# thisparticle/scl_slam

Hardware: AMD Instinct MI355X
Metric: loop-closure candidates/sec: (scan, keyframe) pairs taken through full-database ARG-MIN detection per second (every pair aligned exactly and bounded by the f16 matrix-core screening; only the survivors get the f64 distance), batches of 16 scans, 10k-keyframe DB per GPU (higher is better)
Workload: dtype f64 results; f16-operand / f32-accumulate MFMA screening + f64 exact pass on the survivors

## Files before the change

profiles/summarize_pmc.py:

```python
import collections
import csv
import glob
import json
import sys


def summarize(root, needle):
    agg = collections.defaultdict(list)
    for f in glob.glob(f"{root}/**/*_counter_collection.csv", recursive=True):
        for row in csv.DictReader(open(f)):
            if needle in row["Kernel_Name"]:
                agg[row["Counter_Name"]].append(float(row["Counter_Value"]))
    summary = {k: {"launches": len(v), "mean_per_launch": sum(v) / len(v)} for k, v in sorted(agg.items())}
    res = {"kernel_filter": needle, "counters": summary}
    if "FETCH_SIZE" in summary and "WRITE_SIZE" in summary:
        fetch = summary["FETCH_SIZE"]["mean_per_launch"] * 1024.0 * 2.0
        write = summary["WRITE_SIZE"]["mean_per_launch"] * 1024.0
        res["hbm_bytes_per_launch"] = fetch + write
        res["hbm_read_bytes_corrected_x2"] = fetch
        res["hbm_write_bytes"] = write
    return res


def main():
    root, out = sys.argv[1], sys.argv[2]
    needles = (sys.argv[3] if len(sys.argv) > 3 else "sc_distance").split(",")
    if len(needles) == 1:
        res = summarize(root, needles[0])
    else:
        parts = [summarize(root, n) for n in needles]
        res = {"kernel_filter": needles, "kernels": parts}
        if all("hbm_bytes_per_launch" in p for p in parts):
            res["hbm_bytes_per_launch"] = sum(p["hbm_bytes_per_launch"] for p in parts)
            res["hbm_read_bytes_corrected_x2"] = sum(p["hbm_read_bytes_corrected_x2"] for p in parts)
            res["hbm_write_bytes"] = sum(p["hbm_write_bytes"] for p in parts)
    json.dump(res, open(out, "w"), indent=1)
    print(json.dumps(res, indent=1))


if __name__ == "__main__":
    main()
# ... 1 lines not shown
```

scl_slam_amd/csrc/engine.hip:

```cpp
#include "scl_engine.h"

#include <hip/hip_runtime.h>

#include <cfloat>
#include <climits>
#include <chrono>
#include <cmath>
#include <cstdio>
#include <cstdlib>
#include <cstring>
#include <mutex>
#include <new>
#include <string>
#include <atomic>
#include <chrono>
#include <thread>
#include <vector>

#include "db_file.hpp"
#include "engine_internal.hpp"
#include "device_sort.hpp"
#include "plugin_host.hpp"

#ifdef SCL_DIAGNOSTICS
// ... 451 lines not shown
    if (!c) return SCL_ERR_INVALID_ARG;
    c->num_ring = 20; c->num_sector = 60; c->num_candidates = 3;
    c->dist_thres = 0.14; c->lidar_height = 1.65; c->max_radius = 80.0;
    c->num_exclude_recent = 100; c->tree_making_period = 10;
    c->search_ratio = 0.1;
    c->knn_exclude_eps = 0.0f;
    c->device = 0;
    c->initial_capacity = 4096;
    return SCL_OK;
}

static void log_env_overrides_once()
{
    static std::atomic<bool> done{false};
    if (done.exchange(true)) return;
    static const char *const names[] = {"SCL_SCREEN", "SCL_SCREEN_FORM", "SCL_SCREEN_V2_MIN", "SCL_RCCL_LIB",
                                        "SCL_SCREEN_VARIANT", "SCL_SCREEN_PROBE", "SCL_SCREEN_TAIL", "SCL_ALIGN_WGS",
                                        "SCL_ALIGN2_WGS", "SCL_ALIGN_FILTER", "SCL_SC_KERNEL", "SCL_SC_WAVES", "SCL_STAMP", "SCL_ABLATE",
                                        "SCL_ICP_REDUCE", "SCL_MATRIX_PLAIN", "SCL_MATRIX_KERNEL", "SCL_MATRIX_KR", "SCL_WIDE_EXACT", "SCL_STREAM_EXACT", "SCL_SMALL_EXACT_OFF",
                                        "SCL_SELF_ALIGN_OFF", "SCL_CAND_EXACT_OFF"};
    constexpr int kProduct = 4;
    int i = 0;
    for (const char *n : names) {
        const char *v = getenv(n);
#ifdef SCL_DIAGNOSTICS
        if (v) fprintf(stderr, "scl_engine (diagnostics build): environment override in effect: %s=%s\n", n, v);
#else
        if (v && i < kProduct) fprintf(stderr, "scl_engine: environment override in effect: %s=%s\n", n, v);
        else if (v) fprintf(stderr, "scl_engine: %s=%s is an experiment's switch: ignored by this build (make EXTRA=-DSCL_DIAGNOSTICS builds them in)\n", n, v);
#endif
        ++i;
    }
    (void)kProduct;
}

int scl_create(const scl_config *cfg, scl_engine **out)
// ... 779 lines not shown
int scl_sc_search_inter(scl_engine *e, const int *curs, int count, int robot_pre, int k, int *cand_ids, int *cand_shifts, double *cand_dists,
                        int *n_found)
{
    if (!e || count < 0 || k < 1 || k > SCL_SC_SEARCH_MAX || (count > 0 && (!curs || !cand_ids))) return SCL_ERR_INVALID_ARG;
    if (robot_pre < SCL_SC_ANY_OTHER_ROBOT || robot_pre > 127) return SCL_ERR_INVALID_ARG;
    if (count == 0) return SCL_OK;
    if (e->front) return front_sc_search_inter(e, curs, count, robot_pre, k, cand_ids, cand_shifts, cand_dists, n_found);
    return sc_search_robot(e, curs, count, true, robot_pre, k, cand_ids, cand_shifts, cand_dists, n_found);
}

namespace {

int submit_full_many_locked(scl_engine *e, const int *queries, const int *los, const int *his, int nq, int *tickets);

struct ScreenGroup { const int *qslot, *lo, *n; int nq, set0; int part_half = 0; bool masks = false; bool keys_later = false; };
int launch_screen_group(scl_engine *e, const ScreenGroup &cur, int phases = kScreenAlign | kScreenProducts,
                        const ScreenGroup *next = nullptr, hipStream_t stream = nullptr)
{
    if (!stream) stream = e->stream;
    auto fill = [&](ScreenBatch &sb, const ScreenGroup &g) {
        sb.nq = g.nq;
        for (int j = 0; j < g.nq; ++j) { sb.slot[j] = g.qslot[j]; sb.base[j] = g.lo[j]; sb.n[j] = g.n[j]; sb.buf[j] = g.set0 + j; }
        sb.pair_stride = e->set_stride;
        sb.approx = e->d_approx; sb.starts = e->d_starts; sb.align_fallbacks = e->d_align_fallbacks; sb.ring_d2 = e->d_ring_d2;
        sb.survivors = nullptr; sb.n_surv = nullptr; sb.t_min = e->d_tmin;
        sb.smask = (g.masks || sc_screen_is_wide(db_view(e), e->SR)) ? e->d_smask : nullptr;
        sb.part = e->d_part + (g.part_half ? e->part_cap / 2 : 0);
        sb.no_ring_metric = g.keys_later;
        sb.k = e->cfg.num_candidates; sb.exclude_eps = e->cfg.knn_exclude_eps; sb.topk_idx = e->d_topk_idx; sb.topk_d2 = e->d_topk_d2;
    };
    ScreenBatch sb{}, nx{};
    fill(sb, cur);
    const bool has_next = next && next->nq > 0;
    if (has_next) fill(nx, *next);
    if (phases & kScreenAlign) for (int j = 0; j < cur.nq; ++j) e->align_pairs += (uint64_t)cur.n[j];
    if (has_next) for (int j = 0; j < next->nq; ++j) e->align_pairs += (uint64_t)next->n[j];
    if ((phases & kScreenAlign) && (phases & kScreenProducts) && has_next) {
        SCL_HIP(e, launch_sc_screen_batch(db_view(e), sb, e->SR, sc_align_filter_enabled(), e->num_cu, stream, kScreenAlign, nullptr));
        phases = kScreenProducts;
    }
    ProfScope ps(e, P_SC, stream);
    SCL_HIP(e, launch_sc_screen_batch(db_view(e), sb, e->SR, sc_align_filter_enabled(), e->num_cu, stream, phases, has_next ? &nx : nullptr));
    if (ps.active()) { for (int j = 0; j < cur.nq; ++j) e->prof.sc_distance_pairs += (uint64_t)cur.n[j]; }
    return SCL_OK;
}

unsigned survivor_arg_region(scl_engine *e) { return e->surv_arg_tick++ & 7u; }
int launch_survivor_pass(scl_engine *e, const int *qslot, const int *lo, const int *n, int nq, int set0, double *const *out3, hipStream_t stream = nullptr,
                         int phases = kSurvivorArgs | kSurvivorKernel, int region_in = -1, bool ring_from_keys = false)
{
    if (!stream) stream = e->stream;
    SurvivorPass sp{};
    sp.nq = nq; sp.ring_from_keys = ring_from_keys ? 1 : 0;
    for (int j = 0; j < nq; ++j) { sp.slot[j] = qslot[j]; sp.base[j] = lo[j]; sp.n[j] = n[j]; sp.buf[j] = set0 + j; sp.out3[j] = out3[j]; }
    sp.pair_stride = e->set_stride;
    sp.approx = e->d_approx; sp.survivors = e->d_surv; sp.t_min = e->d_tmin; sp.out_dist = e->d_dist; sp.out_shift = e->d_shift;
    sp.blk_part = e->d_surv_part; sp.done_counter = e->d_surv_done; sp.surv_stats = e->d_surv_stats;
    sp.ring_d2 = e->d_ring_d2; sp.k = e->cfg.num_candidates; sp.exclude_eps = e->cfg.knn_exclude_eps; sp.topk_idx = e->d_topk_idx; sp.topk_d2 = e->d_topk_d2;
// ... 366 lines not shown

int stream_screened_locked(scl_engine *e, std::unique_lock<std::mutex> &db, const int *queries, const int *lo, const int *hi, int n_queries, int spl,
                           int *nn_idx, int *shift, double *dist)
{
    const int n0 = e->n;
    constexpr int NS = scl_engine::kScreenSets;
    constexpr int CH = NS / 2;
    static_assert(CH <= kMaxSurvivorQueries, "one exact pass takes the survivors of a whole chunk");
    const bool wide = sc_screen_is_wide(db_view(e), e->SR);
#ifndef SCL_WIDE_CHUNK
#define SCL_WIDE_CHUNK 64
#endif
    const int chmax = wide && CH > SCL_WIDE_CHUNK ? SCL_WIDE_CHUNK : CH;
    const int chn = spl >= 1 && spl <= chmax ? (chmax / spl) * spl : chmax;
    struct List { int qslot[CH], qlo[CH], qn[CH], pos[CH], m = 0; };
    struct Chunk { int first = 0, count = 0; bool busy = false, aligned = false, small = false; std::vector<int> lo, empty; };
    Chunk ch[2];
    bool sub0_valid[2] = {false, false};
    const bool small_exact = sc_small_exact_supported(db_view(e), e->SR) && (!wide || e->d_smask) && !scl_lab_is("SCL_STREAM_EXACT", "s");
    const bool keys_later = !wide && !small_exact;
    int nmax = 1;
    for (int i = 0; i < n_queries; ++i) {
        const int l = lo[i] < 0 ? 0 : lo[i], h = hi[i] > n0 ? n0 : hi[i];
        if (h - l > nmax) nmax = h - l;
    }
    int rc = ensure_sets(e, (size_t)nmax);
    if (rc) return rc;
    SCL_HIP(e, hipEventRecord(e->ev_align_gate, e->stream));
    SCL_HIP(e, hipStreamWaitEvent(e->stream_surv, e->ev_align_gate, 0));
    auto build = [&](int first, int count, List &L, Chunk *k) -> int {
        L.m = 0;
        for (int i = 0; i < count; ++i) {
            const int q = queries[first + i];
            int slot;
            if (q >= 0) { if (q >= n0) return fail(e, SCL_ERR_OUT_OF_RANGE, "query slot out of range"); slot = q; }
// ... 27 lines not shown
        if (e->prof_on == 3 && cur.m > 0) {
            if ((e->prof_tick++ & 1) == 0) {
                auto get = [&]() { hipEvent_t ev = nullptr; if (!e->event_pool.empty()) { ev = e->event_pool.back(); e->event_pool.pop_back(); } else if (hipEventCreate(&ev) != hipSuccess) ev = nullptr; return ev; };
                span_start = get(); span_stop = get();
                if (span_start && span_stop) (void)hipEventRecord(span_start, e->stream); else { span_start = span_stop = nullptr; }
            }
            e->prof_on = 0;
        }
        auto span_end = [&]() {
            if (!span_start) return;
            (void)hipEventRecord(span_stop, e->stream);
            e->pending.push_back({span_start, span_stop, P_SC, span_groups});
            for (int j = 0; j < cur.m; ++j) e->prof.sc_distance_pairs += (uint64_t)cur.qn[j];
            span_start = nullptr;
        };
        bool next_aligned = false;
        for (int g = 0; g < cur.m; g += spl) {
            const int w = cur.m - g < spl ? cur.m - g : spl;
            ScreenGroup grp{cur.qslot + g, cur.qlo + g, cur.qn + g, w, set0 + g};
            grp.keys_later = keys_later;
            ScreenGroup nx{nullptr, nullptr, nullptr, 0, 0};
            if (g + w < cur.m) {
                const int wn = cur.m - g - w < spl ? cur.m - g - w : spl;
                nx = ScreenGroup{cur.qslot + g + w, cur.qlo + g + w, cur.qn + g + w, wn, set0 + g + w};
                nx.keys_later = keys_later;
            } else if (ncount > 0 && nxt.m > 0) {
                const int wn = nxt.m < spl ? nxt.m : spl;
                nx = ScreenGroup{nxt.qslot, nxt.qlo, nxt.qn, wn, nset0};
                nx.keys_later = keys_later;
                if (ch[c ^ 1].busy) SCL_HIP(e, hipStreamWaitEvent(e->stream, (wide && sub0_valid[c ^ 1] && wn <= kWideExactBatch) ? e->ev_sub0[c ^ 1] : e->ev_chunk[c ^ 1], 0));
                next_aligned = true;
            }
            const int phases = (g == 0 && !k.aligned) ? (kScreenAlign | kScreenProducts) : kScreenProducts;
            if ((rc = launch_screen_group(e, grp, phases, nx.nq > 0 ? &nx : nullptr))) return rc;
            ++span_groups;
        }
        span_end();
        hipStream_t xs = ncount > 0 ? e->stream_surv : e->stream;
        if (ncount > 0) {
            SCL_HIP(e, hipEventRecord(e->ev_k1[c], e->stream));
            SCL_HIP(e, hipStreamWaitEvent(e->stream_surv, e->ev_k1[c], 0));
        } else if (cur.m > 0) {
            if (hipEventQuery(e->ev_k1[c]) != hipSuccess) SCL_HIP(e, hipStreamWaitEvent(e->stream, e->ev_k1[c], 0));
        }
        sub0_valid[c] = wide && !k.small && cur.m > 0;
        if (cur.m > 0 && (rc = k.small ? launch_small_exact_chunk(e, cur.qslot, cur.qlo, cur.qn, cur.m, set0, out3, xs, kSurvivorKernel, region)
                             : wide ? launch_survivor_pass_wide(e, cur.qslot, cur.qlo, cur.qn, cur.m, set0, out3, xs, e->ev_sub0[c])
                                    : launch_survivor_pass(e, cur.qslot, cur.qlo, cur.qn, cur.m, set0, out3, xs, kSurvivorKernel, region, keys_later))) return rc;
        SCL_HIP(e, hipEventRecord(e->ev_chunk[c], xs));
        k.busy = true;
        k.aligned = false;
        ch[c ^ 1].aligned = next_aligned;
        e->last_pass_empty = cur.m == 0;
        return SCL_OK;
    };
    auto collect = [&](int c, bool last) -> int {
        Chunk &k = ch[c];
        auto wait_chunk = [&]() -> hipError_t {
            hipError_t q;
            const auto t0 = std::chrono::steady_clock::now();
            int spins = 0;
            while ((q = hipEventQuery(e->ev_chunk[c])) == hipErrorNotReady) {
                for (int p = 0; p < 32; ++p) cpu_relax();
                if ((++spins & 255) == 0 && std::chrono::steady_clock::now() - t0 > std::chrono::milliseconds(20)) return hipEventSynchronize(e->ev_chunk[c]);
            }
            return q;
// ... 2253 lines not shown
```

scl_slam_amd/csrc/kernels.hpp:

```cpp
#pragma once

#include <hip/hip_runtime.h>
#include <stdint.h>

#include <stdlib.h>

namespace scl {

#ifdef SCL_DIAGNOSTICS
inline int scl_lab_int(const char *name, int dflt) { const char *e = getenv(name); return e ? atoi(e) : dflt; }
inline bool scl_lab_is(const char *name, const char *value) { const char *e = getenv(name); if (!e) return false; while (*value) if (*e++ != *value++) return false; return true; }
#else
constexpr int scl_lab_int(const char *, int dflt) { return dflt; }
constexpr bool scl_lab_is(const char *, const char *) { return false; }
#endif

constexpr double kBigDist = 10000000.0;
constexpr int kTminEpsOffset = 256;
constexpr int hdesc_sector(int RG) { return ((RG * 8 + 63) / 64) * 8; }
constexpr int hkey_halfs(int S) { return ((S + 31) / 32) * 32; }
constexpr int hkey_store_halfs(int S) { return hkey_halfs(S) + 8; }
constexpr int hkey_row_halfs(int S) { return 2 * hkey_halfs(S) + 8; }
constexpr int halign_P(int S) { return S % 8 == 0 ? 8 : (S % 4 == 0 ? 4 : 0); }
constexpr int halign_CP(int S) { return ((S + 8 + 31) / 32) * 32; }
// ... 116 lines not shown
    unsigned long long *align_fallbacks;
    unsigned long long *surv_stats;
    unsigned int *smask;
    int k; float exclude_eps; int *topk_idx; float *topk_d2;
    float *part;
    bool no_ring_metric;
};
bool sc_screen_supported(const struct DbView &db, int SR);
bool sc_screen_is_wide(const struct DbView &db, int SR);
float sc_screen_eps();
int sc_screen_max_batch(const struct DbView &db, int SR);
size_t sc_screen_scratch_floats(const struct DbView &db, int SR);
constexpr int kScreenAlign = 1, kScreenProducts = 2;
hipError_t launch_sc_screen_batch(const struct DbView &db, const ScreenBatch &sb, int SR, int align_filter, int num_cu, hipStream_t stream,
                                  int phases = kScreenAlign | kScreenProducts, const ScreenBatch *next = nullptr);
hipError_t launch_sc_select_batch(const ScreenBatch &sb, hipStream_t stream);
constexpr int kSurvivorBlocks = 2;
constexpr int kSurvivorArgBytes = 384;
constexpr int kMaxSurvivorQueries = 128;
struct SurvivorPass {
    int nq;
    int slot[kMaxSurvivorQueries], base[kMaxSurvivorQueries], n[kMaxSurvivorQueries], buf[kMaxSurvivorQueries];
    double *out3[kMaxSurvivorQueries];
    size_t pair_stride;
    const float *approx; int *survivors; unsigned int *t_min; double *out_dist; int *out_shift;
    const float *ring_d2; int k; float exclude_eps; int *topk_idx; float *topk_d2;
    unsigned long long *blk_part; unsigned int *done_counter;
    unsigned long long *surv_stats;
    void *d_args; void *h_args;
    int ring_from_keys;
// ... 62 lines not shown
```

scl_slam_amd/csrc/sc_screen.hip:

```cpp
#include <atomic>
#include <type_traits>

#include "align_exact.hpp"
#include "device_common.hpp"
#include "kernels.hpp"

namespace scl {

namespace {

typedef _Float16 h4 __attribute__((ext_vector_type(4)));
typedef _Float16 h8 __attribute__((ext_vector_type(8)));
typedef float f4v __attribute__((ext_vector_type(4)));
typedef float f2 __attribute__((ext_vector_type(2)));
typedef unsigned int u32x4 __attribute__((ext_vector_type(4)));
typedef u32x4 __attribute__((aligned(8))) u32x4_a8;

struct ScreenArgs {
    const double *vkey;
    const uint2 *hdesc; const unsigned int *kmask;
    const double *q_vkey; const float *q_rkey;
    const uint2 *q_hdesc; const unsigned int *q_kmask;
    const _Float16 *hkey; const _Float16 *q_hkey; int hkw;
    const float4 *rkey4; int rk_cap;
// ... 947 lines not shown
    using C = S2Cfg<RG, S, W>;
    return (size_t)(C::NQ / (4 * C::SPK)) * s2_quad(S, C::STEPS * C::SPK, C::SPK);
}
template <int RG, int S, int W> constexpr bool s2_group_used(int p, int g4) { return 4 * g4 < kS2PassRows && W - 1 - S2Cfg<RG, S, W>::PS * p - 4 * g4 >= 0; }
template <int RG, int S, int W> constexpr int s2_pass_f4(int p) { int n = 0; for (int g = 0; g < 4; ++g) n += s2_group_used<RG, S, W>(p, g) ? 1 : 0; return n; }
template <int RG, int S, int W> constexpr int s2_pass_off(int p) { int o = 0; for (int q = 0; q < p; ++q) o += s2_pass_f4<RG, S, W>(q); return o; }
template <int RG, int S, int W> constexpr int s2_part_f4() { return s2_pass_off<RG, S, W>(S2Cfg<RG, S, W>::NPASS); }
template <int RG, int S, int W> constexpr int s2_part_floats() { return S2Cfg<RG, S, W>::NP * s2_part_f4<RG, S, W>() * 4; }

struct Screen2Args {
    ScreenBatchArgs prod;
    float *part;
    int u_lo, u_n;
    int nwg;
};

template <int RG, int S, int W>
__global__ __launch_bounds__((S2Cfg<RG, S, W>::WV * kWave), 1) void sc_screen2_kernel(Screen2Args fa)
{
    using C = S2Cfg<RG, S, W>;
    constexpr int WVP = C::WV;
    constexpr int NP = C::NP, NPASS = C::NPASS, STEPS = C::STEPS, NQ = C::NQ, SPK = C::SPK, PS = C::PS;
    constexpr bool AOFF = PS != kS2PassRows;
    constexpr int NB = AOFF ? 1 : NPASS;
    constexpr int LAG = AOFF ? PS / 4 : 0;
    constexpr int RGH = hdesc_rgh(RG);
    constexpr int SB = RGH * 8;
    constexpr int HS = hdesc_stride(RG, S);
    constexpr int SECT = STEPS * SPK;
    constexpr int NIT = S / SECT;
    constexpr int ROWS = S + SECT - 1;
    constexpr int QUAD = s2_quad(S, SECT, SPK);
    constexpr int SPR = 4 * SPK, SCB = 64 / SPK;
    static_assert(SB >= SCB * NP && SB == 64 * ((NP * SCB + 63) / 64) && S % SECT == 0 && SECT == 4 && kS2PassRows + SPK * (STEPS - 1) <= 16 && W <= PS * (NPASS - 1) + kS2PassRows && (!AOFF || (NPASS == 2 && PS == 12))
                  && NQ % SPR == 0 && NQ <= kMaxScreenBatch && (SPK == 1 || SPK == 2), "second form");
    static_assert(SPK == 2 ? QUAD % 256 == 0 : (QUAD / 16) % 4 == 2, "bank slots of the image's blocks");
    extern __shared__ __attribute__((aligned(16))) unsigned char smem2[];
    const ScreenBatchArgs &ab = fa.prod;
    const int lane = threadIdx.x & (kWave - 1);
    const int wave = __builtin_amdgcn_readfirstlane((int)(threadIdx.x >> 6));
    const int b = (int)blockIdx.x, xcd = b & 7, jx = b >> 3;
    const int part = jx % NP;
    const int gi = (jx / NP) * 8 + xcd;
    const int waves_part = (fa.nwg / NP) * WVP;
    const int gw = gi * WVP + wave;

#ifdef S2_STAMP
#define S2_STAMP_AT(slot) do { if ((wave == 0 || wave == 5) && (b == 0 || b == 37) && lane == 0) g_s2_stamps[((b ? 2 : 0) + (wave ? 1 : 0)) * 64 + (slot)] = __builtin_amdgcn_s_memtime(); } while (0)
#else
#define S2_STAMP_AT(slot) do { } while (0)
#endif
    S2_STAMP_AT(32);
    const int c16 = lane & 15, j4 = lane >> 4;
    const int cq = c16 < NQ ? c16 : c16 - 12;
    const ScreenQuery sq = ab.q[cq];
    const int *starts_q = ab.starts + (size_t)sq.buf * (size_t)ab.pair_stride;
    const bool q_live = c16 < ab.nq && c16 < NQ;
    const int lsec = c16 + (SPK == 2 ? (j4 >> 1) : 0);
    const unsigned int a_lane = (unsigned int)(hdesc2_offset(RG, S) * 8 + (((SPK == 2 ? part * 2 + (j4 & 1) : part * 4 + j4)) * (S + 16) + lsec) * 16);
    const unsigned char *hd = reinterpret_cast<const unsigned char *>(ab.hdesc);
// ... 207 lines not shown
#pragma unroll
            for (int p = 0; p < NPASS; ++p) {
                f4v sum = acc[p][0];
#pragma unroll
                for (int u = 1; u < STEPS; ++u) {
                    constexpr int kMaxSh = SPK * (STEPS - 1);
                    const int sh = SPK * u;
                    float nx[4];
#pragma unroll
                    for (int e2 = 0; e2 < kMaxSh; ++e2)
                        if (e2 < sh) nx[e2] = __int_as_float(__builtin_amdgcn_ds_bpermute(up16, __float_as_int(acc[p][u][e2])));
#pragma unroll
                    for (int i = 0; i < 4; ++i) sum[i] += (i + sh <= 3) ? acc[p][u][(i + sh) & 3] : nx[(i + sh - 4) & 3];
                }
                if (ok && j4 < s2_pass_f4<RG, S, W>(p))
                    *reinterpret_cast<f4v *>(fa.part + (((size_t)c16 * (size_t)ab.pair_stride + (size_t)ci) * NP + part) * (s2_part_f4<RG, S, W>() * 4) + (s2_pass_off<RG, S, W>(p) + j4) * 4) = sum;
            }
        }
        base_cur = base_nxt; base_nxt = kf_base(k + 2);
        b_cur = b_nxt; b_nxt = first_shift(k + 2);
        if (k < 6) S2_STAMP_AT(36 + 3 * k);
    }
    S2_STAMP_AT(60);
}

template <int S>
__device__ __forceinline__ void build_rotq(const unsigned int *q_kmask, uint4 *rotq, int tid, int nthreads)
{
    constexpr int NW64 = (S + 63) / 64, MW = (NW64 + 1) / 2;
    unsigned long long qm[NW64];
#pragma unroll
// ... 222 lines not shown
    if (b < align_blocks) {
        const int wave = __builtin_amdgcn_readfirstlane((int)(threadIdx.x >> 6));
        sc_align2_role<S, W>(nb, halign, u_lo, u_n, b * kScreenWaves + wave, align_blocks * kScreenWaves, smem_tail2 + (size_t)wave * Align2Cfg<S>::LDS_WAVE);
        return;
    }
    int qi, chunk;
    if (!finish_block_of(b - align_blocks, fa.prod.nq, chunks, qi, chunk)) return;
    sc_screen2_finish_body<RG, S, W, MASKS, D2>(fa, qi, chunk);
}

static bool screen_second_form()
{
    static const int form = [] { const char *e = getenv("SCL_SCREEN_FORM"); return e ? atoi(e) : 2; }();
    return form != 1;
}
static int screen_v2_min_env()
{
    static const int v = [] { const char *e = getenv("SCL_SCREEN_V2_MIN"); return e ? atoi(e) : 0; }();
    return v;
}
int sc_screen_max_batch(const DbView &db, int SR)
{
    return (sc_screen_is_wide(db, SR) && screen_second_form()) ? S2Cfg<20, 180, 19>::NQ : kMaxScreenBatch;
}
size_t sc_screen_scratch_floats(const DbView &db, int SR)
{
    return sc_screen_is_wide(db, SR) ? (size_t)S2Cfg<20, 180, 19>::NQ * s2_part_floats<20, 180, 19>() : (size_t)S2Cfg<16, 120, 13>::NQ * s2_part_floats<16, 120, 13>();
}

static int fill_screen_args(const DbView &db, const ScreenBatch &sb, int align_filter, ScreenBatchArgs *ab)
// ... 1 lines not shown
    ab->vkey = db.vkey; ab->rkey = db.rkey; ab->hdesc = db.hdesc; ab->kmask = db.kmask; ab->rkey4 = db.rkey4; ab->hkey = db.hkey; ab->hkw = hkey_row_halfs(db.S);
    ab->starts = sb.starts; ab->approx = sb.approx; ab->ring_d2 = sb.ring_d2; ab->t_min = sb.t_min; ab->fallbacks = sb.align_fallbacks; ab->smask = sb.smask;
    ab->pair_stride = (unsigned long long)sb.pair_stride;
    ab->S = db.S; ab->R4 = 4 * db.RG; ab->hstride = db.hstride; ab->rk_cap = db.cap; ab->align_filter = align_filter;
    ab->nq = sb.nq;
    int nmax = 0;
    for (int i = 0; i < sb.nq; ++i) {
        if (sb.n[i] <= 0) return -1;
        ab->q[i] = ScreenQuery{sb.slot[i], sb.base[i], sb.n[i], sb.buf[i]};
        nmax = sb.n[i] > nmax ? sb.n[i] : nmax;
    }
    for (int i = sb.nq; i < kMaxScreenBatch; ++i) ab->q[i] = ab->q[0];
    return nmax;
}

template <int RG, int S, int W, int OCC0, int OCC1>
static hipError_t launch_screen_grid(const DbView &db, const ScreenBatch &sb, int align_filter, int num_cu, hipStream_t stream, int phases,
                                     const ScreenBatch *next)
{
    constexpr int RGH = hdesc_rgh(RG);
    ScreenBatchArgs ab{};
    const int nmax = fill_screen_args(db, sb, align_filter, &ab);
    if (nmax < 0) return hipErrorInvalidValue;
    const int ngroups = (nmax + kGroup - 1) / kGroup;
    static_assert(halign_bytes(S) > 0, "alignment image");
    if (db.hstride != hdesc_stride(RG, S) || !sb.starts || !db.halign) return hipErrorInvalidValue;
    static std::atomic<bool> attr_set_dev[64];
    int dev_ = 0; (void)hipGetDevice(&dev_);
    std::atomic<bool> &attr_set = attr_set_dev[dev_ & 63];
    static const int variant = scl_lab_int("SCL_SCREEN_VARIANT", 0);
    void (*kern)(ScreenFusedArgs) = sc_screen_kernel<RG, S, W, 15, OCC0>;
#ifdef SCL_DIAGNOSTICS
    if (variant == 1) kern = sc_screen_kernel<RG, S, W, 15, OCC1>;
    if (variant == 2) kern = sc_screen_kernel<RG, S, W, 5, OCC0>;
    static const int probe = scl_lab_int("SCL_SCREEN_PROBE", 0);
    if (probe == 2) kern = sc_screen_kernel<RG, S, W, 15, OCC0, 2>;
#else
    const int probe = 0;
// ... 16 lines not shown
    }
    auto align_blocks = [&](int groups, int nq, bool beside_products) {
        int b = (groups + kScreenWaves - 1) / kScreenWaves;
        static const int cap_env = scl_lab_int("SCL_ALIGN_WGS", 0);
        int cap = cap_env > 0 ? cap_env : (beside_products ? 2 * num_cu / (nq > 0 ? nq : 1) : num_cu);
        if (cap < 1) cap = 1;
        return b > cap ? cap : b;
    };
    const int v2_min = screen_v2_min_env() > 0 ? screen_v2_min_env() : (S <= 128 ? 4 : 2);
    auto second_form_for = [&](const ScreenBatch &b) {
        return screen_second_form() && b.part && probe == 0 && variant == 0 && b.nq >= v2_min && b.nq <= S2Cfg<RG, S, W>::NQ;
    };
    const bool use_v2 = second_form_for(sb);
    const bool next_v2 = next && second_form_for(*next);
    ab.skip_d2 = use_v2 ? 1 : 0;
    constexpr size_t lds_a2 = (size_t)kScreenWaves * Align2Cfg<S>::LDS_WAVE;
    auto union_of = [](const ScreenBatch &b, int *lo_out, int *n_out) {
        int lo = b.base[0], hi = b.base[0] + b.n[0];
        for (int i = 1; i < b.nq; ++i) { lo = b.base[i] < lo ? b.base[i] : lo; hi = b.base[i] + b.n[i] > hi ? b.base[i] + b.n[i] : hi; }
        *lo_out = lo; *n_out = hi - lo;
    };
    auto align2_blocks = [&](int u_n) {
        static const int env = scl_lab_int("SCL_ALIGN2_WGS", 0);
        int b = (u_n + kScreenWaves * 3 - 1) / (kScreenWaves * 3);
        const int cap = env > 0 ? env : 2 * num_cu;
        b = b > cap ? cap : b;
        return b < 1 ? 1 : b;
    };
    const bool self_align = (phases & kScreenAlign) && (phases & kScreenProducts) && !use_v2 && probe == 0 && !scl_lab_int("SCL_SELF_ALIGN_OFF", 0);
    if ((phases & kScreenAlign) && probe != 3 && !self_align) {
// ... 5 lines not shown
            ab.nb = align_blocks(ngroups, sb.nq, false);
            hipLaunchKernelGGL((sc_align_kernel<RG, S, W>), dim3(ab.nb * sb.nq), dim3(kScreenWaves * kWave), lds0, stream, ab);
        }
        hipError_t e = hipGetLastError();
        if (e != hipSuccess) return e;
    }
    if (probe == 4 || !(phases & kScreenProducts)) return hipSuccess;
    if (use_v2) {
        static std::atomic<bool> attr2_dev[64];
        std::atomic<bool> &attr2 = attr2_dev[dev_ & 63];
        if (!attr2.load(std::memory_order_acquire)) {
            hipError_t e = hipFuncSetAttribute((const void *)sc_screen2_kernel<RG, S, W>, hipFuncAttributeMaxDynamicSharedMemorySize, (int)(s2_lds<RG, S, W>()));
            if (e != hipSuccess) return e;
            attr2.store(true, std::memory_order_release);
        }
        Screen2Args f2{};
        f2.prod = ab; f2.part = sb.part;
        union_of(sb, &f2.u_lo, &f2.u_n);
        constexpr int WGU = 8 * S2Cfg<RG, S, W>::NP;
        int nwg = (num_cu / WGU) * WGU;
        if (nwg < WGU) nwg = WGU;
        f2.nwg = nwg;
        hipError_t e = hipSuccess;
        hipLaunchKernelGGL((sc_screen2_kernel<RG, S, W>), dim3(nwg), dim3(S2Cfg<RG, S, W>::WV * kWave), (s2_lds<RG, S, W>()), stream, f2);
        if ((e = hipGetLastError()) != hipSuccess) return e;
        const int chunks = (nmax + 255) / 256;
        const dim3 fgrid(finish_blocks(chunks, sb.nq)), ablock(kScreenWaves * kWave);
        if (!next) {
            hipLaunchKernelGGL((sc_screen2_finish_kernel<RG, S, W>), fgrid, dim3(256), 0, stream, f2, chunks);
            return hipGetLastError();
        }
        if (next->nq < 1 || next->nq > kMaxScreenBatch) return hipErrorInvalidValue;
        ScreenBatchArgs nb{};
        const int nmax2 = fill_screen_args(db, *next, align_filter, &nb);
        if (nmax2 < 0) return hipErrorInvalidValue;
        nb.skip_d2 = next_v2 ? 1 : 0;
        int ulo = 0, un = 0, ablocks;
        if (next_v2) {
            union_of(*next, &ulo, &un);
            ablocks = align2_blocks(un);
        } else {
            const int ng2 = (nmax2 + kGroup - 1) / kGroup;
            int per_q = 3 * num_cu / next->nq;
            per_q = per_q < 1 ? 1 : per_q;
            nb.nb = (ng2 + kScreenWaves - 1) / kScreenWaves;
            nb.nb = nb.nb > per_q ? per_q : nb.nb;
            ablocks = nb.nb * next->nq;
        }
        static const int tail_env = scl_lab_int("SCL_SCREEN_TAIL", 1);
        if (tail_env) {
            const dim3 tgrid(ablocks + finish_blocks(chunks, sb.nq));
            const bool d2 = !sb.no_ring_metric;
            if (!next_v2) hipLaunchKernelGGL((sc_screen2_tail_kernel<RG, S, W>), tgrid, ablock, lds0, stream, f2, nb, ablocks, chunks);
            else if (sb.smask && d2) hipLaunchKernelGGL((sc_screen2_tail2_kernel<RG, S, W, true, true>), tgrid, ablock, lds_a2, stream, f2, nb, db.halign, ulo, un, ablocks, chunks);
            else if (sb.smask) hipLaunchKernelGGL((sc_screen2_tail2_kernel<RG, S, W, true, false>), tgrid, ablock, lds_a2, stream, f2, nb, db.halign, ulo, un, ablocks, chunks);
            else if (d2) hipLaunchKernelGGL((sc_screen2_tail2_kernel<RG, S, W, false, true>), tgrid, ablock, lds_a2, stream, f2, nb, db.halign, ulo, un, ablocks, chunks);
            else hipLaunchKernelGGL((sc_screen2_tail2_kernel<RG, S, W, false, false>), tgrid, ablock, lds_a2, stream, f2, nb, db.halign, ulo, un, ablocks, chunks);
            return hipGetLastError();
        }
        hipLaunchKernelGGL((sc_screen2_finish_kernel<RG, S, W>), fgrid, dim3(256), 0, stream, f2, chunks);
        if ((e = hipGetLastError()) != hipSuccess) return e;
        if (next_v2) hipLaunchKernelGGL((sc_align2_kernel<RG, S, W>), dim3(ablocks), ablock, lds_a2, stream, nb, db.halign, ulo, un);
        else hipLaunchKernelGGL((sc_align_kernel<RG, S, W>), dim3(ablocks), ablock, lds0, stream, nb);
        return hipGetLastError();
    }
    ScreenFusedArgs fa{};
    fa.prod = ab;
    int blocks = num_cu * 2;
    if (blocks > ngroups) blocks = ngroups;
    if (blocks > kScreenMaxBlocks) blocks = kScreenMaxBlocks;
    fa.prod.nb = blocks;
    fa.prod.self_align = self_align ? 1 : 0;
    int extra = 0;
    if (next && probe != 3) {
        if (next->nq < 1 || next->nq > kMaxScreenBatch) return hipErrorInvalidValue;
        const int nmax2 = fill_screen_args(db, *next, align_filter, &fa.next);
        if (nmax2 < 0) return hipErrorInvalidValue;
        fa.next.skip_d2 = next_v2 ? 1 : 0;
        fa.next.nb = align_blocks((nmax2 + kGroup - 1) / kGroup, next->nq, true);
// ... 7 lines not shown
    const int patterned = fused_patterned_blocks(sb.nq, blocks, extra);
    const int slots = 8 * ((blocks + 7) >> 3);
    const int grid = patterned + (extra > slots ? extra - slots : 0);
    hipLaunchKernelGGL(kern, dim3(grid), dim3(kScreenWaves * kWave), lds, stream, fa);
    return hipGetLastError();
}

hipError_t launch_sc_screen_batch(const DbView &db, const ScreenBatch &sb, int SR, int align_filter, int num_cu, hipStream_t stream, int phases,
                                  const ScreenBatch *next)
{
    if (sb.nq < 1 || sb.nq > kMaxScreenBatch || !sc_screen_supported(db, SR)) return hipErrorInvalidValue;
    if (sc_screen_is_wide(db, SR)) return launch_screen_grid<20, 180, 19, 2, 2>(db, sb, align_filter, num_cu, stream, phases, next);
    return launch_screen_grid<16, 120, 13, 2, 3>(db, sb, align_filter, num_cu, stream, phases, next);
}

}

#ifdef S2_STAMP
extern "C" int scl_debug_s2_stamps(unsigned long long *out)
{
    return (int)hipMemcpyFromSymbol(out, HIP_SYMBOL(scl::g_s2_stamps), sizeof(unsigned long long) * 4 * 64);
}
#endif
```

Before: 2.465 billion.

## Screen two full scan batches in one paired second-form products launch

Adds a paired variant of the second-form screening kernel that processes two full 16-scan batches in one grid, splitting workgroups across the two sets and writing to separate halves of the partial buffer. The chunk loop now walks groups in pairs when both are full, aligns ahead up to two groups, and tracks alignment progress as a count instead of a boolean. The aim is to amortise launch and keyframe-streaming cost across twice as many scans per pass over the database. In exchange, each set gets half the workgroups, and the alignment and next-group bookkeeping becomes more complex.

```diff
diff --git a/profiles/summarize_pmc.py b/profiles/summarize_pmc.py
--- a/profiles/summarize_pmc.py
+++ b/profiles/summarize_pmc.py
@@ -9,7 +9,7 @@
     agg = collections.defaultdict(list)
     for f in glob.glob(f"{root}/**/*_counter_collection.csv", recursive=True):
         for row in csv.DictReader(open(f)):
-            if needle in row["Kernel_Name"]:
+            if needle.replace(" ", "") in row["Kernel_Name"].replace(" ", ""):
                 agg[row["Counter_Name"]].append(float(row["Counter_Value"]))
     summary = {k: {"launches": len(v), "mean_per_launch": sum(v) / len(v)} for k, v in sorted(agg.items())}
     res = {"kernel_filter": needle, "counters": summary}
@@ -24,7 +24,8 @@
 
 def main():
     root, out = sys.argv[1], sys.argv[2]
-    needles = (sys.argv[3] if len(sys.argv) > 3 else "sc_distance").split(",")
+    needles = sys.argv[3] if len(sys.argv) > 3 else "sc_distance"
+    needles = [n for n in needles.split(";" if ";" in needles else ",") if n]
     if len(needles) == 1:
         res = summarize(root, needles[0])
     else:
diff --git a/scl_slam_amd/csrc/engine.hip b/scl_slam_amd/csrc/engine.hip
--- a/scl_slam_amd/csrc/engine.hip
+++ b/scl_slam_amd/csrc/engine.hip
@@ -489,12 +489,12 @@
 {
     static std::atomic<bool> done{false};
     if (done.exchange(true)) return;
-    static const char *const names[] = {"SCL_SCREEN", "SCL_SCREEN_FORM", "SCL_SCREEN_V2_MIN", "SCL_RCCL_LIB",
+    static const char *const names[] = {"SCL_SCREEN", "SCL_SCREEN_FORM", "SCL_SCREEN_V2_MIN", "SCL_SCREEN_PAIR", "SCL_RCCL_LIB",
                                         "SCL_SCREEN_VARIANT", "SCL_SCREEN_PROBE", "SCL_SCREEN_TAIL", "SCL_ALIGN_WGS",
                                         "SCL_ALIGN2_WGS", "SCL_ALIGN_FILTER", "SCL_SC_KERNEL", "SCL_SC_WAVES", "SCL_STAMP", "SCL_ABLATE",
                                         "SCL_ICP_REDUCE", "SCL_MATRIX_PLAIN", "SCL_MATRIX_KERNEL", "SCL_MATRIX_KR", "SCL_WIDE_EXACT", "SCL_STREAM_EXACT", "SCL_SMALL_EXACT_OFF",
                                         "SCL_SELF_ALIGN_OFF", "SCL_CAND_EXACT_OFF"};
-    constexpr int kProduct = 4;
+    constexpr int kProduct = 5;
     int i = 0;
     for (const char *n : names) {
         const char *v = getenv(n);
@@ -1304,25 +1304,27 @@
 int submit_full_many_locked(scl_engine *e, const int *queries, const int *los, const int *his, int nq, int *tickets);
 
 struct ScreenGroup { const int *qslot, *lo, *n; int nq, set0; int part_half = 0; bool masks = false; bool keys_later = false; };
+void fill_screen_batch(scl_engine *e, ScreenBatch &sb, const ScreenGroup &g)
+{
+    sb.nq = g.nq;
+    for (int j = 0; j < g.nq; ++j) { sb.slot[j] = g.qslot[j]; sb.base[j] = g.lo[j]; sb.n[j] = g.n[j]; sb.buf[j] = g.set0 + j; }
+    sb.pair_stride = e->set_stride;
+    sb.approx = e->d_approx; sb.starts = e->d_starts; sb.align_fallbacks = e->d_align_fallbacks; sb.ring_d2 = e->d_ring_d2;
+    sb.survivors = nullptr; sb.n_surv = nullptr; sb.t_min = e->d_tmin;
+    sb.smask = (g.masks || sc_screen_is_wide(db_view(e), e->SR)) ? e->d_smask : nullptr;
+    sb.part = e->d_part + (g.part_half ? e->part_cap / 2 : 0);
+    sb.no_ring_metric = g.keys_later;
+    sb.k = e->cfg.num_candidates; sb.exclude_eps = e->cfg.knn_exclude_eps; sb.topk_idx = e->d_topk_idx; sb.topk_d2 = e->d_topk_d2;
+}
+
 int launch_screen_group(scl_engine *e, const ScreenGroup &cur, int phases = kScreenAlign | kScreenProducts,
                         const ScreenGroup *next = nullptr, hipStream_t stream = nullptr)
 {
     if (!stream) stream = e->stream;
-    auto fill = [&](ScreenBatch &sb, const ScreenGroup &g) {
-        sb.nq = g.nq;
-        for (int j = 0; j < g.nq; ++j) { sb.slot[j] = g.qslot[j]; sb.base[j] = g.lo[j]; sb.n[j] = g.n[j]; sb.buf[j] = g.set0 + j; }
-        sb.pair_stride = e->set_stride;
-        sb.approx = e->d_approx; sb.starts = e->d_starts; sb.align_fallbacks = e->d_align_fallbacks; sb.ring_d2 = e->d_ring_d2;
-        sb.survivors = nullptr; sb.n_surv = nullptr; sb.t_min = e->d_tmin;
-        sb.smask = (g.masks || sc_screen_is_wide(db_view(e), e->SR)) ? e->d_smask : nullptr;
-        sb.part = e->d_part + (g.part_half ? e->part_cap / 2 : 0);
-        sb.no_ring_metric = g.keys_later;
-        sb.k = e->cfg.num_candidates; sb.exclude_eps = e->cfg.knn_exclude_eps; sb.topk_idx = e->d_topk_idx; sb.topk_d2 = e->d_topk_d2;
-    };
     ScreenBatch sb{}, nx{};
-    fill(sb, cur);
+    fill_screen_batch(e, sb, cur);
     const bool has_next = next && next->nq > 0;
-    if (has_next) fill(nx, *next);
+    if (has_next) fill_screen_batch(e, nx, *next);
     if (phases & kScreenAlign) for (int j = 0; j < cur.nq; ++j) e->align_pairs += (uint64_t)cur.n[j];
     if (has_next) for (int j = 0; j < next->nq; ++j) e->align_pairs += (uint64_t)next->n[j];
     if ((phases & kScreenAlign) && (phases & kScreenProducts) && has_next) {
@@ -1332,6 +1334,27 @@
     ProfScope ps(e, P_SC, stream);
     SCL_HIP(e, launch_sc_screen_batch(db_view(e), sb, e->SR, sc_align_filter_enabled(), e->num_cu, stream, phases, has_next ? &nx : nullptr));
     if (ps.active()) { for (int j = 0; j < cur.nq; ++j) e->prof.sc_distance_pairs += (uint64_t)cur.n[j]; }
+    return SCL_OK;
+}
+
+int launch_screen_pair_group(scl_engine *e, ScreenGroup g0, ScreenGroup g1, bool align0, bool align1, const ScreenGroup *next0, const ScreenGroup *next1)
+{
+    hipStream_t stream = e->stream;
+    g0.part_half = 0; g1.part_half = 1;
+    ScreenBatch sb0{}, sb1{}, nx0{}, nx1{};
+    fill_screen_batch(e, sb0, g0);
+    fill_screen_batch(e, sb1, g1);
+    const bool has0 = next0 && next0->nq > 0, has1 = next1 && next1->nq > 0;
+    if (has0) fill_screen_batch(e, nx0, *next0);
+    if (has1) fill_screen_batch(e, nx1, *next1);
+    const ScreenGroup *counted[4] = {align0 ? &g0 : nullptr, align1 ? &g1 : nullptr, has0 ? next0 : nullptr, has1 ? next1 : nullptr};
+    for (const ScreenGroup *g : counted)
+        if (g) for (int j = 0; j < g->nq; ++j) e->align_pairs += (uint64_t)g->n[j];
+    if (align0) SCL_HIP(e, launch_sc_screen_batch(db_view(e), sb0, e->SR, sc_align_filter_enabled(), e->num_cu, stream, kScreenAlign, nullptr));
+    if (align1) SCL_HIP(e, launch_sc_screen_batch(db_view(e), sb1, e->SR, sc_align_filter_enabled(), e->num_cu, stream, kScreenAlign, nullptr));
+    ProfScope ps(e, P_SC, stream);
+    SCL_HIP(e, launch_sc_screen_pair(db_view(e), sb0, sb1, e->SR, sc_align_filter_enabled(), e->num_cu, stream, has0 ? &nx0 : nullptr, has1 ? &nx1 : nullptr));
+    if (ps.active()) { for (int j = 0; j < g0.nq; ++j) e->prof.sc_distance_pairs += (uint64_t)g0.n[j] + (uint64_t)g1.n[j]; }
     return SCL_OK;
 }
 
@@ -1728,11 +1751,12 @@
     const int chmax = wide && CH > SCL_WIDE_CHUNK ? SCL_WIDE_CHUNK : CH;
     const int chn = spl >= 1 && spl <= chmax ? (chmax / spl) * spl : chmax;
     struct List { int qslot[CH], qlo[CH], qn[CH], pos[CH], m = 0; };
-    struct Chunk { int first = 0, count = 0; bool busy = false, aligned = false, small = false; std::vector<int> lo, empty; };
+    struct Chunk { int first = 0, count = 0; int aligned = 0; bool busy = false, small = false; std::vector<int> lo, empty; };
     Chunk ch[2];
     bool sub0_valid[2] = {false, false};
     const bool small_exact = sc_small_exact_supported(db_view(e), e->SR) && (!wide || e->d_smask) && !scl_lab_is("SCL_STREAM_EXACT", "s");
     const bool keys_later = !wide && !small_exact;
+    const bool pairs = !wide && sc_screen_pairs(db_view(e), e->SR);
     int nmax = 1;
     for (int i = 0; i < n_queries; ++i) {
         const int l = lo[i] < 0 ? 0 : lo[i], h = hi[i] > n0 ? n0 : hi[i];
@@ -1790,27 +1814,42 @@
             for (int j = 0; j < cur.m; ++j) e->prof.sc_distance_pairs += (uint64_t)cur.qn[j];
             span_start = nullptr;
         };
-        bool next_aligned = false;
-        for (int g = 0; g < cur.m; g += spl) {
-            const int w = cur.m - g < spl ? cur.m - g : spl;
-            ScreenGroup grp{cur.qslot + g, cur.qlo + g, cur.qn + g, w, set0 + g};
-            grp.keys_later = keys_later;
-            ScreenGroup nx{nullptr, nullptr, nullptr, 0, 0};
-            if (g + w < cur.m) {
-                const int wn = cur.m - g - w < spl ? cur.m - g - w : spl;
-                nx = ScreenGroup{cur.qslot + g + w, cur.qlo + g + w, cur.qn + g + w, wn, set0 + g + w};
-                nx.keys_later = keys_later;
-            } else if (ncount > 0 && nxt.m > 0) {
-                const int wn = nxt.m < spl ? nxt.m : spl;
-                nx = ScreenGroup{nxt.qslot, nxt.qlo, nxt.qn, wn, nset0};
-                nx.keys_later = keys_later;
-                if (ch[c ^ 1].busy) SCL_HIP(e, hipStreamWaitEvent(e->stream, (wide && sub0_valid[c ^ 1] && wn <= kWideExactBatch) ? e->ev_sub0[c ^ 1] : e->ev_chunk[c ^ 1], 0));
-                next_aligned = true;
+        auto group_at = [&](int off) {
+            ScreenGroup g{nullptr, nullptr, nullptr, 0, 0};
+            if (off < cur.m) {
+                g = ScreenGroup{cur.qslot + off, cur.qlo + off, cur.qn + off, cur.m - off < spl ? cur.m - off : spl, set0 + off};
+            } else if (ncount > 0 && off - cur.m < nxt.m) {
+                const int o = off - cur.m;
+                g = ScreenGroup{nxt.qslot + o, nxt.qlo + o, nxt.qn + o, nxt.m - o < spl ? nxt.m - o : spl, nset0 + o};
             }
-            const int phases = (g == 0 && !k.aligned) ? (kScreenAlign | kScreenProducts) : kScreenProducts;
-            if ((rc = launch_screen_group(e, grp, phases, nx.nq > 0 ? &nx : nullptr))) return rc;
+            g.keys_later = keys_later;
+            return g;
+        };
+        auto pair_at = [&](int off) { return pairs && group_at(off).nq == kMaxScreenBatch && group_at(off + kMaxScreenBatch).nq == kMaxScreenBatch &&
+                                             (off + 2 * kMaxScreenBatch <= cur.m || off >= cur.m); };
+        int aligned_to = k.aligned;
+        for (int g = 0; g < cur.m;) {
+            const bool pair = pair_at(g);
+            const ScreenGroup g0 = group_at(g), g1 = pair ? group_at(g + g0.nq) : ScreenGroup{nullptr, nullptr, nullptr, 0, 0};
+            const int end = g + g0.nq + g1.nq;
+            ScreenGroup n0{nullptr, nullptr, nullptr, 0, 0}, n1 = n0;
+            if (end >= aligned_to) {
+                n0 = group_at(end);
+                if (pair && pair_at(end)) n1 = group_at(end + n0.nq);
+            }
+            const int reach = end + n0.nq + n1.nq;
+            if (reach > cur.m && n0.nq > 0) {
+                if (ch[c ^ 1].busy) SCL_HIP(e, hipStreamWaitEvent(e->stream, (wide && sub0_valid[c ^ 1] && reach - cur.m <= kWideExactBatch) ? e->ev_sub0[c ^ 1] : e->ev_chunk[c ^ 1], 0));
+            }
+            const bool align0 = g >= aligned_to, align1 = pair && g + g0.nq >= aligned_to;
+            if (pair) rc = launch_screen_pair_group(e, g0, g1, align0, align1, n0.nq > 0 ? &n0 : nullptr, n1.nq > 0 ? &n1 : nullptr);
+            else rc = launch_screen_group(e, g0, align0 ? (kScreenAlign | kScreenProducts) : kScreenProducts, n0.nq > 0 ? &n0 : nullptr);
+            if (rc) return rc;
+            if (reach > aligned_to) aligned_to = reach;
             ++span_groups;
-        }
+            g = end;
+        }
+        const int next_aligned = aligned_to > cur.m ? aligned_to - cur.m : 0;
         span_end();
         hipStream_t xs = ncount > 0 ? e->stream_surv : e->stream;
         if (ncount > 0) {
@@ -1825,7 +1864,7 @@
                                     : launch_survivor_pass(e, cur.qslot, cur.qlo, cur.qn, cur.m, set0, out3, xs, kSurvivorKernel, region, keys_later))) return rc;
         SCL_HIP(e, hipEventRecord(e->ev_chunk[c], xs));
         k.busy = true;
-        k.aligned = false;
+        k.aligned = 0;
         ch[c ^ 1].aligned = next_aligned;
         e->last_pass_empty = cur.m == 0;
         return SCL_OK;
diff --git a/scl_slam_amd/csrc/kernels.hpp b/scl_slam_amd/csrc/kernels.hpp
--- a/scl_slam_amd/csrc/kernels.hpp
+++ b/scl_slam_amd/csrc/kernels.hpp
@@ -154,6 +154,9 @@
 constexpr int kScreenAlign = 1, kScreenProducts = 2;
 hipError_t launch_sc_screen_batch(const struct DbView &db, const ScreenBatch &sb, int SR, int align_filter, int num_cu, hipStream_t stream,
                                   int phases = kScreenAlign | kScreenProducts, const ScreenBatch *next = nullptr);
+bool sc_screen_pairs(const struct DbView &db, int SR);
+hipError_t launch_sc_screen_pair(const struct DbView &db, const ScreenBatch &sb0, const ScreenBatch &sb1, int SR, int align_filter, int num_cu,
+                                 hipStream_t stream, const ScreenBatch *next0, const ScreenBatch *next1);
 hipError_t launch_sc_select_batch(const ScreenBatch &sb, hipStream_t stream);
 constexpr int kSurvivorBlocks = 2;
 constexpr int kSurvivorArgBytes = 384;
diff --git a/scl_slam_amd/csrc/sc_screen.hip b/scl_slam_amd/csrc/sc_screen.hip
--- a/scl_slam_amd/csrc/sc_screen.hip
+++ b/scl_slam_amd/csrc/sc_screen.hip
@@ -985,11 +985,20 @@
     int u_lo, u_n;
     int nwg;
 };
-
-template <int RG, int S, int W>
-__global__ __launch_bounds__((S2Cfg<RG, S, W>::WV * kWave), 1) void sc_screen2_kernel(Screen2Args fa)
+struct Screen2PairArgs {
+    ScreenBatchArgs prod[2];
+    float *part[2];
+    int u_lo, u_n;
+    int nwg;
+};
+template <int NS> struct S2KernelArgs { using type = Screen2Args; };
+template <> struct S2KernelArgs<2> { using type = Screen2PairArgs; };
+
+template <int RG, int S, int W, int NS = 1>
+__global__ __launch_bounds__((S2Cfg<RG, S, W>::WV * kWave), 1) void sc_screen2_kernel(typename S2KernelArgs<NS>::type fa)
 {
     using C = S2Cfg<RG, S, W>;
+    static_assert(NS == 1 || NS == 2, "scan sets of a products launch");
     constexpr int WVP = C::WV;
     constexpr int NP = C::NP, NPASS = C::NPASS, STEPS = C::STEPS, NQ = C::NQ, SPK = C::SPK, PS = C::PS;
     constexpr bool AOFF = PS != kS2PassRows;
@@ -1007,14 +1016,18 @@
                   && NQ % SPR == 0 && NQ <= kMaxScreenBatch && (SPK == 1 || SPK == 2), "second form");
     static_assert(SPK == 2 ? QUAD % 256 == 0 : (QUAD / 16) % 4 == 2, "bank slots of the image's blocks");
     extern __shared__ __attribute__((aligned(16))) unsigned char smem2[];
-    const ScreenBatchArgs &ab = fa.prod;
     const int lane = threadIdx.x & (kWave - 1);
     const int wave = __builtin_amdgcn_readfirstlane((int)(threadIdx.x >> 6));
     const int b = (int)blockIdx.x, xcd = b & 7, jx = b >> 3;
     const int part = jx % NP;
-    const int gi = (jx / NP) * 8 + xcd;
-    const int waves_part = (fa.nwg / NP) * WVP;
+    const int set = (jx / NP) % NS;
+    const int gi = (jx / (NP * NS)) * 8 + xcd;
+    const int waves_part = (fa.nwg / (NP * NS)) * WVP;
     const int gw = gi * WVP + wave;
+    const ScreenBatchArgs *abp; float *part_out;
+    if constexpr (NS == 2) { abp = set ? &fa.prod[1] : &fa.prod[0]; part_out = set ? fa.part[1] : fa.part[0]; }
+    else { abp = &fa.prod; part_out = fa.part; }
+    const ScreenBatchArgs &ab = *abp;
 
 #ifdef S2_STAMP
 #define S2_STAMP_AT(slot) do { if ((wave == 0 || wave == 5) && (b == 0 || b == 37) && lane == 0) g_s2_stamps[((b ? 2 : 0) + (wave ? 1 : 0)) * 64 + (slot)] = __builtin_amdgcn_s_memtime(); } while (0)
@@ -1252,7 +1265,7 @@
                     for (int i = 0; i < 4; ++i) sum[i] += (i + sh <= 3) ? acc[p][u][(i + sh) & 3] : nx[(i + sh - 4) & 3];
                 }
                 if (ok && j4 < s2_pass_f4<RG, S, W>(p))
-                    *reinterpret_cast<f4v *>(fa.part + (((size_t)c16 * (size_t)ab.pair_stride + (size_t)ci) * NP + part) * (s2_part_f4<RG, S, W>() * 4) + (s2_pass_off<RG, S, W>(p) + j4) * 4) = sum;
+                    *reinterpret_cast<f4v *>(part_out + (((size_t)c16 * (size_t)ab.pair_stride + (size_t)ci) * NP + part) * (s2_part_f4<RG, S, W>() * 4) + (s2_pass_off<RG, S, W>(p) + j4) * 4) = sum;
             }
         }
         base_cur = base_nxt; base_nxt = kf_base(k + 2);
@@ -1505,6 +1518,11 @@
     static const int form = [] { const char *e = getenv("SCL_SCREEN_FORM"); return e ? atoi(e) : 2; }();
     return form != 1;
 }
+static bool screen_pair_enabled()
+{
+    static const int on = [] { const char *e = getenv("SCL_SCREEN_PAIR"); return e ? atoi(e) : 1; }();
+    return on != 0;
+}
 static int screen_v2_min_env()
 {
     static const int v = [] { const char *e = getenv("SCL_SCREEN_V2_MIN"); return e ? atoi(e) : 0; }();
@@ -1536,14 +1554,19 @@
     return nmax;
 }
 
+struct ScreenPairMate { const ScreenBatch *sb; const ScreenBatch *next; };
+
 template <int RG, int S, int W, int OCC0, int OCC1>
 static hipError_t launch_screen_grid(const DbView &db, const ScreenBatch &sb, int align_filter, int num_cu, hipStream_t stream, int phases,
-                                     const ScreenBatch *next)
+                                     const ScreenBatch *next, const ScreenPairMate *mate = nullptr)
 {
     constexpr int RGH = hdesc_rgh(RG);
     ScreenBatchArgs ab{};
     const int nmax = fill_screen_args(db, sb, align_filter, &ab);
     if (nmax < 0) return hipErrorInvalidValue;
+    ScreenBatchArgs ab_m{};
+    const int nmax_m = mate ? fill_screen_args(db, *mate->sb, align_filter, &ab_m) : 0;
+    if (nmax_m < 0) return hipErrorInvalidValue;
     const int ngroups = (nmax + kGroup - 1) / kGroup;
     static_assert(halign_bytes(S) > 0, "alignment image");
     if (db.hstride != hdesc_stride(RG, S) || !sb.starts || !db.halign) return hipErrorInvalidValue;
@@ -1590,6 +1613,11 @@
     const bool use_v2 = second_form_for(sb);
     const bool next_v2 = next && second_form_for(*next);
     ab.skip_d2 = use_v2 ? 1 : 0;
+    ab_m.skip_d2 = 1;
+    constexpr bool kPairGrid = S == 120 && S2Cfg<RG, S, W>::NP == 2;
+    if (mate && !(kPairGrid && screen_pair_enabled() && phases == kScreenProducts && use_v2 && second_form_for(*mate->sb) &&
+                  sb.nq == S2Cfg<RG, S, W>::NQ && mate->sb->nq == S2Cfg<RG, S, W>::NQ && mate->sb->part != sb.part))
+        return hipErrorInvalidValue;
     constexpr size_t lds_a2 = (size_t)kScreenWaves * Align2Cfg<S>::LDS_WAVE;
     auto union_of = [](const ScreenBatch &b, int *lo_out, int *n_out) {
         int lo = b.base[0], hi = b.base[0] + b.n[0];
@@ -1625,55 +1653,79 @@
             if (e != hipSuccess) return e;
             attr2.store(true, std::memory_order_release);
         }
-        Screen2Args f2{};
+        Screen2Args f2{}, f2_m{};
         f2.prod = ab; f2.part = sb.part;
         union_of(sb, &f2.u_lo, &f2.u_n);
-        constexpr int WGU = 8 * S2Cfg<RG, S, W>::NP;
+        const int WGU = 8 * S2Cfg<RG, S, W>::NP * (mate ? 2 : 1);
         int nwg = (num_cu / WGU) * WGU;
         if (nwg < WGU) nwg = WGU;
         f2.nwg = nwg;
         hipError_t e = hipSuccess;
-        hipLaunchKernelGGL((sc_screen2_kernel<RG, S, W>), dim3(nwg), dim3(S2Cfg<RG, S, W>::WV * kWave), (s2_lds<RG, S, W>()), stream, f2);
+        if constexpr (kPairGrid) {
+            if (mate) {
+                static std::atomic<bool> attrp_dev[64];
+                std::atomic<bool> &attrp = attrp_dev[dev_ & 63];
+                if (!attrp.load(std::memory_order_acquire)) {
+                    e = hipFuncSetAttribute((const void *)sc_screen2_kernel<RG, S, W, 2>, hipFuncAttributeMaxDynamicSharedMemorySize, (int)(s2_lds<RG, S, W>()));
+                    if (e != hipSuccess) return e;
+                    attrp.store(true, std::memory_order_release);
+                }
+                f2_m.prod = ab_m; f2_m.part = mate->sb->part; f2_m.nwg = nwg;
+                union_of(*mate->sb, &f2_m.u_lo, &f2_m.u_n);
+                Screen2PairArgs fp{};
+                fp.prod[0] = ab; fp.prod[1] = ab_m; fp.part[0] = sb.part; fp.part[1] = mate->sb->part; fp.nwg = nwg;
+                const int hi0 = f2.u_lo + f2.u_n, hi1 = f2_m.u_lo + f2_m.u_n;
+                fp.u_lo = f2.u_lo < f2_m.u_lo ? f2.u_lo : f2_m.u_lo;
+                fp.u_n = (hi0 > hi1 ? hi0 : hi1) - fp.u_lo;
+                hipLaunchKernelGGL((sc_screen2_kernel<RG, S, W, 2>), dim3(nwg), dim3(S2Cfg<RG, S, W>::WV * kWave), (s2_lds<RG, S, W>()), stream, fp);
+            }
+        }
+        if (!mate) hipLaunchKernelGGL((sc_screen2_kernel<RG, S, W>), dim3(nwg), dim3(S2Cfg<RG, S, W>::WV * kWave), (s2_lds<RG, S, W>()), stream, f2);
         if ((e = hipGetLastError()) != hipSuccess) return e;
-        const int chunks = (nmax + 255) / 256;
-        const dim3 fgrid(finish_blocks(chunks, sb.nq)), ablock(kScreenWaves * kWave);
-        if (!next) {
+        auto launch_tail = [&](const ScreenBatch &sb, const Screen2Args &f2, const int nmax, const ScreenBatch *next) -> hipError_t {
+            const bool next_v2 = next && second_form_for(*next);
+            const int chunks = (nmax + 255) / 256;
+            const dim3 fgrid(finish_blocks(chunks, sb.nq)), ablock(kScreenWaves * kWave);
+            if (!next) {
+                hipLaunchKernelGGL((sc_screen2_finish_kernel<RG, S, W>), fgrid, dim3(256), 0, stream, f2, chunks);
+                return hipGetLastError();
+            }
+            if (next->nq < 1 || next->nq > kMaxScreenBatch) return hipErrorInvalidValue;
+            ScreenBatchArgs nb{};
+            const int nmax2 = fill_screen_args(db, *next, align_filter, &nb);
+            if (nmax2 < 0) return hipErrorInvalidValue;
+            nb.skip_d2 = next_v2 ? 1 : 0;
+            int ulo = 0, un = 0, ablocks;
+            if (next_v2) {
+                union_of(*next, &ulo, &un);
+                ablocks = align2_blocks(un);
+            } else {
+                const int ng2 = (nmax2 + kGroup - 1) / kGroup;
+                int per_q = 3 * num_cu / next->nq;
+                per_q = per_q < 1 ? 1 : per_q;
+                nb.nb = (ng2 + kScreenWaves - 1) / kScreenWaves;
+                nb.nb = nb.nb > per_q ? per_q : nb.nb;
+                ablocks = nb.nb * next->nq;
+            }
+            static const int tail_env = scl_lab_int("SCL_SCREEN_TAIL", 1);
+            if (tail_env) {
+                const dim3 tgrid(ablocks + finish_blocks(chunks, sb.nq));
+                const bool d2 = !sb.no_ring_metric;
+                if (!next_v2) hipLaunchKernelGGL((sc_screen2_tail_kernel<RG, S, W>), tgrid, ablock, lds0, stream, f2, nb, ablocks, chunks);
+                else if (sb.smask && d2) hipLaunchKernelGGL((sc_screen2_tail2_kernel<RG, S, W, true, true>), tgrid, ablock, lds_a2, stream, f2, nb, db.halign, ulo, un, ablocks, chunks);
+                else if (sb.smask) hipLaunchKernelGGL((sc_screen2_tail2_kernel<RG, S, W, true, false>), tgrid, ablock, lds_a2, stream, f2, nb, db.halign, ulo, un, ablocks, chunks);
+                else if (d2) hipLaunchKernelGGL((sc_screen2_tail2_kernel<RG, S, W, false, true>), tgrid, ablock, lds_a2, stream, f2, nb, db.halign, ulo, un, ablocks, chunks);
+                else hipLaunchKernelGGL((sc_screen2_tail2_kernel<RG, S, W, false, false>), tgrid, ablock, lds_a2, stream, f2, nb, db.halign, ulo, un, ablocks, chunks);
+                return hipGetLastError();
+            }
             hipLaunchKernelGGL((sc_screen2_finish_kernel<RG, S, W>), fgrid, dim3(256), 0, stream, f2, chunks);
+            if ((e = hipGetLastError()) != hipSuccess) return e;
+            if (next_v2) hipLaunchKernelGGL((sc_align2_kernel<RG, S, W>), dim3(ablocks), ablock, lds_a2, stream, nb, db.halign, ulo, un);
+            else hipLaunchKernelGGL((sc_align_kernel<RG, S, W>), dim3(ablocks), ablock, lds0, stream, nb);
             return hipGetLastError();
-        }
-        if (next->nq < 1 || next->nq > kMaxScreenBatch) return hipErrorInvalidValue;
-        ScreenBatchArgs nb{};
-        const int nmax2 = fill_screen_args(db, *next, align_filter, &nb);
-        if (nmax2 < 0) return hipErrorInvalidValue;
-        nb.skip_d2 = next_v2 ? 1 : 0;
-        int ulo = 0, un = 0, ablocks;
-        if (next_v2) {
-            union_of(*next, &ulo, &un);
-            ablocks = align2_blocks(un);
-        } else {
-            const int ng2 = (nmax2 + kGroup - 1) / kGroup;
-            int per_q = 3 * num_cu / next->nq;
-            per_q = per_q < 1 ? 1 : per_q;
-            nb.nb = (ng2 + kScreenWaves - 1) / kScreenWaves;
-            nb.nb = nb.nb > per_q ? per_q : nb.nb;
-            ablocks = nb.nb * next->nq;
-        }
-        static const int tail_env = scl_lab_int("SCL_SCREEN_TAIL", 1);
-        if (tail_env) {
-            const dim3 tgrid(ablocks + finish_blocks(chunks, sb.nq));
-            const bool d2 = !sb.no_ring_metric;
-            if (!next_v2) hipLaunchKernelGGL((sc_screen2_tail_kernel<RG, S, W>), tgrid, ablock, lds0, stream, f2, nb, ablocks, chunks);
-            else if (sb.smask && d2) hipLaunchKernelGGL((sc_screen2_tail2_kernel<RG, S, W, true, true>), tgrid, ablock, lds_a2, stream, f2, nb, db.halign, ulo, un, ablocks, chunks);
-            else if (sb.smask) hipLaunchKernelGGL((sc_screen2_tail2_kernel<RG, S, W, true, false>), tgrid, ablock, lds_a2, stream, f2, nb, db.halign, ulo, un, ablocks, chunks);
-            else if (d2) hipLaunchKernelGGL((sc_screen2_tail2_kernel<RG, S, W, false, true>), tgrid, ablock, lds_a2, stream, f2, nb, db.halign, ulo, un, ablocks, chunks);
-            else hipLaunchKernelGGL((sc_screen2_tail2_kernel<RG, S, W, false, false>), tgrid, ablock, lds_a2, stream, f2, nb, db.halign, ulo, un, ablocks, chunks);
-            return hipGetLastError();
-        }
-        hipLaunchKernelGGL((sc_screen2_finish_kernel<RG, S, W>), fgrid, dim3(256), 0, stream, f2, chunks);
-        if ((e = hipGetLastError()) != hipSuccess) return e;
-        if (next_v2) hipLaunchKernelGGL((sc_align2_kernel<RG, S, W>), dim3(ablocks), ablock, lds_a2, stream, nb, db.halign, ulo, un);
-        else hipLaunchKernelGGL((sc_align_kernel<RG, S, W>), dim3(ablocks), ablock, lds0, stream, nb);
-        return hipGetLastError();
+        };
+        if ((e = launch_tail(sb, f2, nmax, next)) != hipSuccess || !mate) return e;
+        return launch_tail(*mate->sb, f2_m, nmax_m, mate->next);
     }
     ScreenFusedArgs fa{};
     fa.prod = ab;
@@ -1711,6 +1763,20 @@
     return launch_screen_grid<16, 120, 13, 2, 3>(db, sb, align_filter, num_cu, stream, phases, next);
 }
 
+bool sc_screen_pairs(const DbView &db, int SR)
+{
+    return sc_screen_supported(db, SR) && !sc_screen_is_wide(db, SR) && screen_second_form() && screen_pair_enabled() && screen_v2_min_env() <= kMaxScreenBatch &&
+           scl_lab_int("SCL_SCREEN_VARIANT", 0) == 0 && scl_lab_int("SCL_SCREEN_PROBE", 0) == 0;
+}
+
+hipError_t launch_sc_screen_pair(const DbView &db, const ScreenBatch &sb0, const ScreenBatch &sb1, int SR, int align_filter, int num_cu, hipStream_t stream,
+                                 const ScreenBatch *next0, const ScreenBatch *next1)
+{
+    if (!sc_screen_pairs(db, SR) || sb0.nq != kMaxScreenBatch || sb1.nq != kMaxScreenBatch) return hipErrorInvalidValue;
+    const ScreenPairMate mate{&sb1, next1};
+    return launch_screen_grid<16, 120, 13, 2, 3>(db, sb0, align_filter, num_cu, stream, kScreenProducts, next0, &mate);
+}
+
 }
 
 #ifdef S2_STAMP
```

After: 2.672 billion, median of 6. +8.4%, better.
